# ORNL/DDStore

Hardware: NVIDIA H100
Metric: batch_fetch_GBps (higher is better)
Workload: dtype u8

## Files before the change

ddstore_b200/csrc/kernels.cu:

```cuda
#include <cuda_runtime.h>
#include <stdint.h>
#include <stdio.h>
#include <stdlib.h>
#include <string.h>

#include <algorithm>
#include <atomic>
#include <type_traits>

#include "kernels.h"

namespace {

thread_local char g_cuda_err[512] = "";
std::atomic<unsigned long long> g_launches{0};

#define CUDA_TRY(expr)                                                                                   \
    do {                                                                                                 \
        cudaError_t e__ = (expr);                                                                        \
        if (e__ != cudaSuccess) {                                                                        \
            snprintf(g_cuda_err, sizeof(g_cuda_err), "%s failed: %s (%s:%d)", #expr, cudaGetErrorString(e__), \
                     __FILE__, __LINE__);                                                                \
            return (int)e__ ? (int)e__ : -1;                                                             \
        }                                                                                                \
// ... 537 lines not shown
            continue;
        }
        src[k] = s;
        nbytes[k] = count[k] * vp[k]->row_bytes;
    }
}

__device__ __forceinline__ int64_t warp_incl_scan(int64_t v, int lane) {
#pragma unroll
    for (int d = 1; d < 32; d <<= 1) {
        int64_t o = __shfl_up_sync(0xffffffffu, v, d);
        if (lane >= d) v += o;
    }
    return v;
}
__device__ __forceinline__ int64_t warp_sum(int64_t v) {
#pragma unroll
    for (int d = 16; d > 0; d >>= 1) v += __shfl_xor_sync(0xffffffffu, v, d);
    return v;
}

constexpr int kFopAdd = 0, kFopSwap = 1, kFopCas = 2;

struct GatherArgs {
    ddsk_var_t var;
    const int64_t *starts;
    int64_t count;
    const uint64_t *req_src;
    const int64_t *req_dst;
    const uint32_t *seg_tab;
    PlanSrc plan;
    int64_t *total_out;
    int64_t nreq;
    char *dst;
    int64_t dst_cap;
    int64_t *offsets_out;
    unsigned long long *status;
    unsigned long long status_tag;
    unsigned int *counters;
    union {
        struct {
            char *mdst[DDSK_MAX_MULTI];
            int64_t mcap[DDSK_MAX_MULTI];
            int64_t *moffsets[DDSK_MAX_MULTI];
        };
        struct {
            int64_t pad_slot;
            uint64_t pad_bits;
// ... 32 lines not shown
    uint32_t n;
    uint32_t off;
};

template <int PCAP>
struct PlanView {
    uint32_t src_s, dst_s;
    __device__ __forceinline__ uint64_t s(int64_t i) const { return lds64(src_s + (uint32_t)i * 8u); }
    __device__ __forceinline__ int64_t d(int64_t i) const { return (int64_t)lds32(dst_s + (uint32_t)i * 4u); }
};
template <>
struct PlanView<0> {
    const uint64_t *src;
    const int64_t *dst;
    const uint32_t *seg_tab;
    __device__ __forceinline__ uint64_t s(int64_t i) const { return __ldcg(&src[i]); }
    __device__ __forceinline__ int64_t d(int64_t i) const { return __ldcg(&dst[i]); }
};

__device__ __forceinline__ void pad_lookup(const GatherArgs &a, int64_t idx, uint64_t &src, int64_t &payload) {
    const int64_t ix[1] = {idx};
    uint64_t s[1];
    int64_t nbytes[1];
    plan_many<1>(a.var, a.plan, ix, a.nreq, a.status, a.status_tag, s, nbytes);
    src = s[0];
    payload = min(nbytes[0], a.pad_slot);
}

__device__ __forceinline__ uint4 pad_pattern(uint64_t bits, int el) {
    uint32_t lo, hi;
    if (el == 0) lo = hi = (uint32_t)(bits & 0xFFu) * 0x01010101u;
    else if (el == 1) lo = hi = (uint32_t)(bits & 0xFFFFu) * 0x00010001u;
    else if (el == 2) lo = hi = (uint32_t)bits;
    else {
        lo = (uint32_t)bits;
        hi = (uint32_t)(bits >> 32);
    }
    return make_uint4(lo, hi, lo, hi);
}
__device__ __forceinline__ void pad_store1(char *d, uint64_t bits, int el) {
    if (el == 0) *(uint8_t *)d = (uint8_t)bits;
    else if (el == 1) *(uint16_t *)d = (uint16_t)bits;
    else if (el == 2) *(uint32_t *)d = (uint32_t)bits;
    else *(uint64_t *)d = bits;
}
__device__ __forceinline__ void pad_fill(char *d, int64_t n, uint64_t bits, int el, int lane) {
    int64_t head = (16 - (int64_t)((uint64_t)d & 15u)) & 15;
// ... 29 lines not shown
    int64_t w_dst = 0, w_n = 0;
    uint64_t w_shard;

    __device__ __forceinline__ void load_window(const GatherArgs &a, int lane) {
        win_base = r;
        int64_t idx = r + lane;
        w_src = 0;
        w_dst = 0;
        w_n = 0;
        if (idx < nreq) {
            if constexpr (PAD) {
                int64_t payload;
                pad_lookup(a, idx, w_src, payload);
                w_dst = idx * nb;
                w_n = payload;
            } else if (FIXED && push_n > 0) {
                int p = 0;
                for (int k = 1; k < push_n; k++)
                    if (idx >= push_rbase[k]) p = k;
                const int64_t i = idx - push_rbase[p];
                const int64_t start = ld_relaxed_sys_s64((const int64_t *)(push_win[p] + push_idx_off) + i);
                uint64_t s = 0;
                int owner = 0;
                const int code = dev_locate_owner(a.var, start, a.count, &s, &owner);
                if (code && owner == push_me) {
                    unsigned long long *st = (unsigned long long *)push_win[p] + 3;
                    asm volatile("red.relaxed.sys.global.min.u64 [%0], %1;" ::"l"(st), "l"(((unsigned long long)i << 8) | (unsigned long long)code) : "memory");
                }
                w_src = (code || owner != push_me) ? 0 : s;
                w_dst = idx * nb;
                w_n = nb;
            } else if (FIXED) {
                uint64_t s = 0;
                int code = dev_locate(a.var, a.starts[idx], a.count, &s);
                if (code) report(a.status, a.status_tag, idx, code);
                w_src = code ? 0 : s;
                w_dst = idx * nb;
                w_n = nb;
            } else {
                w_src = pv.s(idx);
                w_dst = pv.d(idx);
                w_n = pv.d(idx + 1) - w_dst;
            }
            if constexpr (PUT) {
                w_shard = w_src;
                w_src = w_src ? (uint64_t)a.dst + (uint64_t)w_dst : 0;
            }
        }
    }

    __device__ __forceinline__ int64_t align_to_var(int64_t pos) const {
        int64_t b = vb[0];
#pragma unroll
        for (int k = 1; k < (VALIGN ? DDSK_MAX_MULTI : 1); k++)
            if (pos >= vb[k]) b = vb[k];
        return b + ((pos - b) & ~(int64_t)7);
    }
// ... 679 lines not shown

struct NoCvt {
    int32_t unused_;
};
template <bool CVT>
using CvtParam = typename std::conditional<CVT, ddsk_cvt_t, NoCvt>::type;

template <int NW, int PCAP, bool CVT = false, bool NORM = false, bool PUT = false>
__device__ __forceinline__ int64_t plan_in_smem(const GatherArgs &a, const PlanView<PCAP> &pv, int64_t *wtot, int warp,
                                                int lane, bool writer, int code = 0) {
    auto out = [&](int64_t x) -> int64_t {
        if constexpr (CVT) return cvt_scale<NORM>(x, code);
        else return x;
    };
    const int64_t nreq = a.nreq;
    const int64_t per_warp = ((nreq + NW * 128 - 1) / (NW * 128)) * 128;
    const int64_t w0 = min(nreq, (int64_t)warp * per_warp), w1 = min(nreq, w0 + per_warp);
    int64_t lane_sum = 0;
    for (int64_t b = w0; b < w1; b += 128) {
        int64_t idx[4], nb[4];
        uint64_t sv[4];
#pragma unroll
        for (int k = 0; k < 4; k++) idx[k] = b + k * 32 + lane;
        plan_many<4, PUT>(a.var, a.plan, idx, w1, a.status, a.status_tag, sv, nb);
#pragma unroll
        for (int k = 0; k < 4; k++) {
            if (idx[k] < w1) {
                sts64(pv.src_s + (uint32_t)idx[k] * 8u, sv[k]);
                sts32(pv.dst_s + (uint32_t)idx[k] * 4u, (uint32_t)min(nb[k], (int64_t)0xFFFFFFFFll));
                lane_sum += nb[k];
            }
        }
    }
    const int64_t wsum = warp_sum(lane_sum);
    if (lane == 0) wtot[warp] = wsum;
    __syncthreads();
    int64_t mine = lane < NW ? wtot[lane] : 0;
    const int64_t T = warp_sum(mine);
    const int64_t base = warp_sum(lane < warp ? mine : 0);
    int64_t run = base;
    for (int64_t b = w0; b < w1; b += 32) {
        const int64_t i = b + lane;
        const int64_t v = i < w1 ? (int64_t)lds32(pv.dst_s + (uint32_t)i * 4u) : 0;
        const int64_t incl = warp_incl_scan(v, lane);
        if (i < w1) {
            sts32(pv.dst_s + (uint32_t)i * 4u, (uint32_t)(run + incl - v));
            if (writer && a.offsets_out) a.offsets_out[i] = out(run + incl - v);
// ... 41 lines not shown
    static_assert(FIXED || !PAD, "a padded batch is a fixed-stride walk");
    static_assert(!PUT || (!CVT && !PAD), "a put writes raw rows");
    static_assert(PUT || !ACC, "an accumulate is a put that adds");
    static_assert((PUT && !ACC) || !FETCH, "a fetch-op is a put that returns the previous rows");
    constexpr int STAGE = CH + 32;
    constexpr bool PUSH = FIXED && !CVT && !PAD && !PUT;
    extern __shared__ __align__(128) unsigned char smem_dyn[];
    __shared__ __align__(8) uint64_t full_bar[NW][S];
    __shared__ __align__(16) PieceDesc desc[NW][S][32];
    __shared__ int64_t wtot[PCAP > 0 ? NW : 1];
    __shared__ int64_t push_rbase[PUSH ? DDSK_MAX_RANKS + 1 : 1];
    __shared__ uint64_t push_win[PUSH ? DDSK_MAX_RANKS : 1];

    const int lane = threadIdx.x & 31;
    const int warp = threadIdx.x >> 5;
    const int64_t gwarp = (int64_t)blockIdx.x * NW + warp;
    const int64_t nwarps = (int64_t)gridDim.x * NW;

    if (lane == 0) {
#pragma unroll
        for (int s = 0; s < S; s++) mbar_init(smem_u32(&full_bar[warp][s]), 1);
        fence_mbar_init();
    }
    uint32_t lut_s = 0;
    if constexpr (CVT) {
        lut_s = smem_u32(smem_dyn) + (uint32_t)(NW * S * STAGE + (PCAP ? PCAP * 12 + 16 : 0));
        for (int i = threadIdx.x; i < c.lut_bytes / 4; i += NW * 32) sts32(lut_s + 4u * (uint32_t)i, c.lut[i]);
        __syncthreads();
    }
    int code0 = 0;
    if constexpr (CVT) code0 = c.code[0];
    if (a.dbg && threadIdx.x == 0) a.dbg[blockIdx.x * 4 + 0] = globaltimer_ns();
    if (a.overlap && !a.wait1_valid) {
        asm volatile("griddepcontrol.wait;" ::: "memory");
        asm volatile("griddepcontrol.launch_dependents;" ::: "memory");
    } else {
        asm volatile("griddepcontrol.launch_dependents;" ::: "memory");
        if (!a.skip_wait) asm volatile("griddepcontrol.wait;" ::: "memory");
    }
    bool gate_open = !(a.overlap && a.wait2_valid);
    auto pass_gate = [&]() {
        if (!gate_open) {
            if (lane == 0) spin_until_done(a.ovl, a.seq - 2u, a.status, a.status_tag, a.nreq);
            __syncwarp();
            gate_open = true;
        }
    };

    ChunkWalker<FIXED, CH, PCAP, CVT, PAD, PUT> w;
    if (!FIXED) {
        if constexpr (PCAP > 0) {
            w.pv.src_s = smem_u32(smem_dyn) + (uint32_t)(NW * S * STAGE);
// ... 64 lines not shown
                    mine_n = ld_relaxed_sys_s64((const int64_t *)ps->win[r] + 1 + par);
                }
                const int64_t incl = warp_incl_scan(mine_n, lane);
                if (r < P) push_rbase[r] = n + incl - mine_n;
                n += __shfl_sync(0xffffffffu, incl, 31);
            }
            if (lane == 0) push_rbase[P] = n;
        }
        __syncthreads();
        w.push_n = P;
        w.push_me = me;
        w.push_par = par;
        w.push_rbase = push_rbase;
        w.push_win = push_win;
        w.push_idx_off = ps->idx_off[par];
    }
    if (a.dbg && threadIdx.x == 0) a.dbg[blockIdx.x * 4 + 1] = globaltimer_ns();
    bool dbg_first = a.dbg != nullptr && warp == 0;
    w.gwarp = gwarp;
    w.nwarps = nwarps;
    w.static_claims = a.tickets == nullptr;
    w.gate_ok = gate_open;
    if constexpr (PAD) w.nb = a.pad_slot;
    else w.nb = (FIXED && a.count <= a.var.lenlist[a.var.nranks - 1]) ? a.count * a.var.row_bytes : 0;
    w.nreq = (FIXED && push) ? push_rbase[w.push_n] : a.nreq;
    if (FIXED) w.T = w.nb * w.nreq;
    bool over = w.T > a.dst_cap;
    const int64_t push_dst_off = (FIXED && push) ? a.push->dst_off[w.push_par] : 0;
    const bool multi = !FIXED && a.plan.nvars > 1;
    int64_t vbase[DDSK_MAX_MULTI + 1];
#pragma unroll
    for (int v = 0; v <= DDSK_MAX_MULTI; v++) vbase[v] = INT64_MAX;
    if (multi) {
        over = false;
#pragma unroll
        for (int v = 0; v < DDSK_MAX_MULTI; v++)
            if (v < a.plan.nvars) vbase[v] = w.pv.d((int64_t)v * a.plan.per_var);
#pragma unroll
        for (int v = 0; v < DDSK_MAX_MULTI; v++)
            if (v < a.plan.nvars) {
                const int64_t endv = v + 1 < a.plan.nvars ? vbase[v + 1] : w.T;
                over |= endv - vbase[v] > a.mcap[v];
            }
        if (PCAP > 0) over |= w.T > 0xFFFFFFFFll;
        if constexpr (CVT) {
            w.valign = true;
#pragma unroll
// ... 46 lines not shown
    {
        if constexpr (PAD) {
            w.seg_bytes = ddsk_fixed_seg_bytes(w.T, w.nb, nwarps, a.min_seg_chunks, CH);
        } else {
        int64_t target = w.T / (nwarps * 8);
        const int64_t unit = (!FIXED && PCAP == 0) ? SEG_GRAIN : (int64_t)CH;
        target = max((int64_t)a.min_seg_chunks * CH, min(target, (int64_t)1 << 20));
        target = max(target, unit);
        if (FIXED && w.nb > 0 && w.nb <= target)
            w.seg_bytes = (target / w.nb) * w.nb;
        else
            w.seg_bytes = (target / unit) * unit;
        }
        w.nseg = w.T > 0 ? (w.T + w.seg_bytes - 1) / w.seg_bytes : 0;
    }
    if (over) {
        if (gwarp == 0 && lane == 0) report(a.status, a.status_tag, a.nreq, DDSK_CODE_CAPACITY);
        w.nseg = 0;
    }

    if (FIXED && !PAD && !push && (w.nb <= 0 || over)) {
        for (int64_t i = gwarp * 32 + lane; i < a.nreq; i += nwarps * 32) {
            uint64_t s;
            int code = dev_locate(a.var, a.starts[i], a.count, &s);
            if (code) report(a.status, a.status_tag, i, code);
        }
    }

    const uint32_t ring = smem_u32(smem_dyn) + (uint32_t)warp * (uint32_t)(S * STAGE);

    uint32_t issued = 0, consumed = 0;
    bool more = w.nseg > 0;
    while (true) {
        while (more && issued - consumed < (uint32_t)(S - 1)) {
            Piece pc;
            const uint32_t total = w.template next_group<STAGE>(a, lane, pc, pass_gate);
            if (total == 0) {
                more = false;
                break;
            }
            const uint32_t st = issued % S;
            const uint32_t bar = smem_u32(&full_bar[warp][st]);
            bulk_wait_read<1>();
            if (lane == 0) mbar_expect_tx(bar, total);
            __syncwarp();
            const uint32_t al = (uint32_t)(pc.src & 15u);
            desc[warp][st][lane].dpos = pc.dpos;
// ... 145 lines not shown
            if (v < a.plan.nvars && a.moffsets[v]) {
                const int64_t basev = w.pv.d((int64_t)v * a.plan.per_var);
                int64_t e = (v * a.plan.per_var + j == a.nreq) ? w.T : w.pv.d((int64_t)v * a.plan.per_var + j);
                if constexpr (CVT) a.moffsets[v][j] = cvt_scale<NORM>(e - basev, c.code[v]);
                else a.moffsets[v][j] = e - basev;
            }
        }
        if constexpr (CVT) {
            if (gwarp == 0 && lane == 0 && a.total_out) {
                int64_t t = 0;
#pragma unroll
                for (int v = 0; v < DDSK_MAX_MULTI; v++)
                    if (v < a.plan.nvars) t += cvt_scale<NORM>((v + 1 < a.plan.nvars ? vbase[v + 1] : w.T) - vbase[v], c.code[v]);
                *a.total_out = t;
            }
        }
    }
    if constexpr (PAD) {
        if (a.pad_lengths || w.nb == 0) {
            for (int64_t i = gwarp * 32 + lane; i < a.nreq; i += nwarps * 32) {
                uint64_t src;
                int64_t payload;
                pad_lookup(a, i, src, payload);
                if (a.pad_lengths) a.pad_lengths[i] = payload / a.var.row_bytes;
            }
        }
    }
    if (FIXED && a.offsets_out && !push) {
        if constexpr (CVT) {
            for (int64_t i = gwarp * 32 + lane; i <= a.nreq; i += nwarps * 32) a.offsets_out[i] = cvt_scale<NORM>(i * w.nb, code0);
        } else {
            for (int64_t i = gwarp * 32 + lane; i <= a.nreq; i += nwarps * 32) a.offsets_out[i] = i * w.nb;
        }
    }

    if (a.dbg && lane == 0) atomicMax(&a.dbg[blockIdx.x * 4 + 3], (unsigned long long)globaltimer_ns());
    if (a.overlap) {
        if (lane == 0) {
            __threadfence();
            const unsigned int slot = a.seq & 3u;
            const unsigned int done = atomicAdd(&a.ovl[slot], 1u);
            if (done == (unsigned int)(nwarps - 1)) {
                a.ovl[slot] = 0;
                a.ovl[8 + slot] = 0;
                if (a.wait_plan) a.plan_word[slot] = 0;
                if (a.wait1_valid) spin_until_done(a.ovl, a.seq - 1u, a.status, a.status_tag, a.nreq);
                __threadfence();
// ... 431 lines not shown
        cfg.numAttrs = 2;
    }
    g_l2_base = nullptr;
    g_l2_bytes = 0;
    CUDA_TRY(cudaLaunchKernelEx(&cfg, kern, args...));
    g_launches++;
    return 0;
}

template <bool FIXED, const Geometry &G, const Geometry &GF>
int launch_kind(const GatherArgs &args, cudaStream_t stream, const ddsk_cvt_t *cvt, bool put, bool acc, bool fop) {
    if (fop) return launch_gather_t<FIXED, GF, false, false, false, true, false, true>(args, stream);
    if (acc) return launch_gather_t<FIXED, G, false, false, false, true, true>(args, stream);
    if (put) return launch_gather_t<FIXED, G, false, false, false, true>(args, stream);
    if (cvt) return cvt_has_norm(cvt) ? launch_gather_t<FIXED, G, true, true>(args, stream, cvt)
                                      : launch_gather_t<FIXED, G, true>(args, stream, cvt);
    return launch_gather_t<FIXED, G>(args, stream);
}

template <bool FIXED>
int launch_gather(const GatherArgs &args, cudaStream_t stream, const ddsk_cvt_t *cvt, bool put = false, bool acc = false,
                  bool fop = false) {
    if constexpr (FIXED) {
        const int64_t request_bytes = args.count < ((int64_t)1 << 20) ? args.count * args.var.row_bytes : INT64_MAX;
        if (!put && !acc && !fop && !cvt && request_bytes < 2048) return launch_gather_t<true, kSmallRows>(args, stream);
    }
    return launch_kind<FIXED, kLargeRows, kFetch>(args, stream, cvt, put, acc, fop);
}

int select_s(int64_t nreq, int64_t cap, const ddsk_cvt_t *cvt) {
    if (!g_smem_plan || cap >= ((int64_t)1 << 32) || nreq > kPlanSmemMax || nreq > g_plan_smem_default) return -1;
    if (nreq <= kPlan4K.pcap) return !cvt || cvt_s_fits_t<kPlan4K>(cvt->lut_bytes) ? 0 : -1;
    return !cvt || cvt_s_fits_t<kPlan8K>(cvt->lut_bytes) ? 1 : -1;
}

int gather_args(GatherArgs &a, const ddsk_var_t *var, const ddsk_scratch_t *scr, int flags) {
    if (int rc = pick_geometry()) return rc;
    memset(&a, 0, sizeof(a));
    a.var = *var;
    a.status = scr->status;
    a.status_tag = scr->status_tag;
    a.counters = scr->counters;
    a.host_mirror = (flags & DDSK_F_MIRROR) ? scr->host_mirror : nullptr;
    a.min_seg_chunks = 1;
    a.overlap = (flags & DDSK_F_OVERLAP) ? 1 : 0;
    a.skip_wait = (flags & DDSK_F_SKIP_WAIT) ? 1 : 0;
    a.wait1_valid = (flags & DDSK_F_PREV1) ? 1 : 0;
    a.wait2_valid = (flags & DDSK_F_PREV2) ? 1 : 0;
    a.seq = scr->ovl_seq;
    a.ovl = scr->ovl;
    a.tickets = a.overlap ? nullptr : scr->counters;
    if (flags & (DDSK_F_ACC | DDSK_F_FOP)) a.acc_type = DDSK_F_ACC_TYPE(flags);
    if (flags & DDSK_F_FOP) {
        a.fop_op = (flags & DDSK_F_FOP_CAS) ? kFopCas : (flags & DDSK_F_FOP_SWAP) ? kFopSwap : kFopAdd;
        a.fop_result = (char *)scr->fop_result;
        a.fop_compare = (const char *)scr->fop_compare;
        a.fop_el = DDSK_F_ACC_TYPE(flags);
    }
    return 0;
}

}
// ... 276 lines not shown
```

ddstore_b200/csrc/kernels.h:

```cpp
#ifndef DDSK_KERNELS_H
#define DDSK_KERNELS_H

#include <stdint.h>

#ifdef __cplusplus
extern "C" {
#endif

#define DDSK_MAX_RANKS 64
#define DDSK_MAX_MULTI 4

typedef struct ddsk_var {
    const void *bases[DDSK_MAX_RANKS];
    int64_t lenlist[DDSK_MAX_RANKS];
    int64_t row_bytes;
    int32_t nranks;
    int32_t pad_;
} ddsk_var_t;

#define DDSK_STATUS_OK 0xFFFFFFFFFFFFFFFFull
#define DDSK_STATUS_ORD_SHIFT 48
#define DDSK_STATUS_REQ_MASK 0xFFFFFFFFFFull
#define DDSK_CODE_START 2
#define DDSK_CODE_COUNT 3
#define DDSK_CODE_CAPACITY 12
#define DDSK_CODE_WATCHDOG 14
#define DDSK_CODE_SAMPLE 15

typedef struct ddsk_scratch {
    unsigned long long *status;
    int64_t *total;
    unsigned int *counters;
    unsigned int *ovl;
    unsigned long long *plan_word;
    unsigned int ovl_seq;
    unsigned long long status_tag;
    uint64_t *req_src;
    int64_t *req_dst;
    int64_t *tile_sums;
    unsigned int plan_tag;
// ... 184 lines not shown
```

ddstore_b200/csrc/store.cpp:

```cpp
#include <cuda_runtime_api.h>
#include <sched.h>
#include <sys/random.h>
#include <unistd.h>

#include <algorithm>
#include <atomic>
#include <condition_variable>
#include <mutex>
#include <thread>
#include <cstdio>
#include <cstdlib>
#include <cstring>
#include <ctime>
#include <map>
#include <set>
#include <string>
#include <vector>

#include "ddstore_b200.h"
#include "internal.h"
#include "kernels.h"
#include "vmm.h"


// ... 137 lines not shown
        src = sp;
        dst = d;
        bytes = n;
        remaining = (int)workers.size();
        gen++;
        cv_go.notify_all();
        cv_done.wait(lk, [&] { return remaining == 0; });
    }
    void stop() {
        {
            std::lock_guard<std::mutex> lk(mu);
            quit = true;
        }
        cv_go.notify_all();
        for (auto &t : workers) t.join();
        workers.clear();
    }
};

struct dds_store {
    dds_comm_t *comm = nullptr;
    int rank = 0, size = 1, device = 0, method = 0;
    cudaStream_t stream = nullptr;
    std::map<std::string, Var> vars;
    std::vector<void *> zombies;
    std::vector<dds_vmm::Block> zombie_blocks;
    unsigned long long token = 0;
    unsigned long long reg_seq = 0;
    ddsk_scratch_t scr;
    int64_t *d_starts = nullptr, *d_counts = nullptr;
    int64_t idx_cap = 0;
    void *d_out = nullptr;
    int64_t out_cap = 0;
    unsigned long long *h_status = nullptr;
    char *h_small = nullptr, *d_small = nullptr;
    struct Queue {
        bool pending = false;
        cudaStream_t pending_stream = nullptr;
        int64_t pending_fixed_total = -1;
        const int64_t *pending_total_ptr = nullptr;
        int pending_cvt = 0;
        bool pending_put = false;
        unsigned int queue_len = 0;
        unsigned int ovl_seq = 1;
        int run_len = 0;
        unsigned long long kept_status = DDSK_STATUS_OK;
        int64_t kept_total = 0;
// ... 205 lines not shown
int entry_var(dds_store *s, const char *name, const int *itemsize, int64_t *total_bytes, int64_t *bad_index, Var **v) {
    clear_error();
    if (bad_index) *bad_index = -1;
    if (total_bytes) *total_bytes = 0;
    if (!s) return fail(DDS_ERR_ARG, "null store");
    *v = find_var(s, name);
    if (!*v) return fail(DDS_ERR_UNKNOWN_VAR, name ? name : "(null)");
    if (itemsize && (*v)->itemsize != *itemsize) return fail(DDS_ERR_DTYPE);
    return DDS_OK;
}

void release_var(Var &v, int rank) {
    for (size_t r = 0; r < v.peer_base.size(); r++) {
        if ((int)r == rank || !v.peer_base[r]) continue;
        if (v.peer_opened[r] == 1) cudaIpcCloseMemHandle(v.peer_base[r]);
        if (v.peer_opened[r] == 2) dds_vmm::release(&v.peer_block[r]);
    }
    v.peer_base.clear();
    v.peer_opened.clear();
    v.peer_block.clear();
}

void free_shard(Var &v) {
    if (v.d_tab) cudaFree(v.d_tab);
    v.d_tab = nullptr;
    if (v.d_norm) cudaFree(v.d_norm);
    v.d_norm = nullptr;
    v.norm_nchan = 0;
    if (v.vmm)
        dds_vmm::release(&v.block);
    else if (v.base)
        cudaFree(v.base);
    v.base = nullptr;
}

int register_var(dds_store *s, const char *name, const void *buffer, int64_t nrows, int disp, int itemsize,
                 int buffer_on_device, bool zero_fill) {
    if (!s || !name) return fail(DDS_ERR_ARG, "null store or name");
    int local_rc = DDS_OK;
    std::string local_err;
    auto note = [&](int rc) {
        if (rc && !local_rc) {
            local_rc = rc;
            local_err = dds_last_error();
        }
    };
// ... 6 lines not shown
    note_cuda(cudaSetDevice(s->device), "cudaSetDevice");
    const bool exists = s->vars.count(name) != 0;
    const unsigned long long seq = s->reg_seq++;

    const size_t payload = local_rc ? 0 : (size_t)nrows * (size_t)disp * (size_t)itemsize;
    size_t alloc = ((payload + 16 + 255) / 256) * 256;
    Var v;
    v.vmm = dds_vmm::available(s->device);
    void *base = nullptr;
    if (!local_rc) {
        if (v.vmm) {
            note(dds_vmm::alloc(s->device, alloc, &v.block));
            if (!local_rc) {
                base = v.block.ptr;
                alloc = v.block.size;
            }
        } else {
            note_cuda(cudaMalloc(&base, alloc), "cudaMalloc (shard)");
            if (local_rc) base = nullptr;
        }
    }
    v.base = base;
    v.bytes = alloc;
    if (base) {
        if (zero_fill || payload == 0) {
            note_cuda(cudaMemsetAsync(base, 0, alloc, s->stream), "cudaMemsetAsync (shard)");
        } else {
            note_cuda(cudaMemsetAsync((char *)base + payload, 0, alloc - payload, s->stream), "cudaMemsetAsync (slack)");
            note_cuda(cudaMemcpyAsync(base, buffer, payload,
                                      buffer_on_device ? cudaMemcpyDeviceToDevice : cudaMemcpyHostToDevice, s->stream),
                      "cudaMemcpyAsync (shard fill)");
        }
        note_cuda(cudaStreamSynchronize(s->stream), "cudaStreamSynchronize (shard fill)");
    }

    PeerRec mine;
    memset(&mine, 0, sizeof(mine));
    mine.nrows = local_rc ? 0 : nrows;
    mine.disp = disp;
    mine.itemsize = itemsize;
    mine.pid = (int32_t)getpid();
    mine.device = s->device;
    mine.raw_ptr = (uint64_t)base;
    mine.host_tag = host_tag();
    mine.alloc_bytes = alloc;
    mine.vmm = v.vmm ? 1 : 0;
    if (s->size > 1 && !v.vmm && base) note_cuda(cudaIpcGetMemHandle(&mine.handle, base), "cudaIpcGetMemHandle");
// ... 97 lines not shown
            if (map_rc) break;
            v.peer_base[(size_t)r] = v.peer_block[(size_t)r].ptr;
            v.peer_opened[(size_t)r] = 2;
        } else {
            v.unprotected_peers = true;
            void *mapped = nullptr;
            cudaError_t e = cudaIpcOpenMemHandle(&mapped, p.handle, cudaIpcMemLazyEnablePeerAccess);
            if (e != cudaSuccess) {
                map_rc = cuda_fail(e, "cudaIpcOpenMemHandle");
                break;
            }
            v.peer_base[(size_t)r] = mapped;
            v.peer_opened[(size_t)r] = 1;
        }
    }
    for (int fd : fds)
        if (fd >= 0) close(fd);
    if (!map_rc && v.vmm) {
        for (int r = 0; r < s->size && !map_rc; r++) {
            const PeerRec &p = all[(size_t)r];
            if (r != s->rank && p.pid == mine.pid && p.device != s->device) map_rc = dds_vmm::grant(&v.block, p.device);
        }
    }
    const std::string keep_err = dds_last_error();
    int brc = dds_comm_barrier(s->comm);

    if (map_rc || bad_disp || bad_item || exists) {
        release_var(v, s->rank);
        if (base) {
            if (v.vmm)
                s->zombie_blocks.push_back(v.block);
            else
                s->zombies.push_back(base);
        }
        if (local_rc) {
            g_err = local_err;
            return local_rc;
        }
        if (map_rc) {
            g_err = keep_err;
            return map_rc;
        }
        if (bad_disp) return fail(DDS_ERR_DISP);
        if (bad_item) return fail(DDS_ERR_DTYPE);
        return fail(DDS_ERR_EXISTS, name);
    }
    memset(&v.kv, 0, sizeof(v.kv));
    for (int r = 0; r < s->size; r++) {
        v.kv.bases[r] = v.peer_base[(size_t)r];
        v.kv.lenlist[r] = v.lenlist[(size_t)r];
    }
    v.kv.row_bytes = (int64_t)disp * (int64_t)itemsize;
    v.kv.nranks = s->size;
    if (s->db_enabled && s->d_vars && s->next_var_id < dds_store::kMaxDbVars) {
        if (cudaMemcpy(&s->d_vars[s->next_var_id], &v.kv, sizeof(ddsk_var_t), cudaMemcpyHostToDevice) == cudaSuccess)
            v.id = s->next_var_id++;
        (void)cudaGetLastError();
    }
    s->vars.emplace(v.name, std::move(v));
    return brc;
}

int64_t sat_mul(int64_t a, int64_t b) {
    int64_t r;
    return __builtin_mul_overflow(a, b, &r) ? INT64_MAX : r;
}
int64_t sat_add(int64_t a, int64_t b) {
    int64_t r;
    return __builtin_add_overflow(a, b, &r) ? INT64_MAX : r;
}

int cvt_in_log2(int code) { return DDSK_CVT_IN_LOG2(code); }
int cvt_out_log2(int code) { return DDSK_CVT_OUT_LOG2(code); }
int64_t cvt_to_out(int64_t p, int code) {
    if (p == INT64_MAX) return p;
    return sat_mul(p >> cvt_in_log2(code), (int64_t)1 << cvt_out_log2(code));
// ... 37 lines not shown
    q.pending = false;
    q.pending_put = false;
    break_run(s);
    cudaStream_t st = q.pending_stream;
    CU(cudaMemcpyAsync(&s->h_status[0], s->scr.status, 8, cudaMemcpyDeviceToHost, st));
    if (q.pending_fixed_total < 0 && q.pending_total_ptr)
        CU(cudaMemcpyAsync(&s->h_status[1], q.pending_total_ptr, 8, cudaMemcpyDeviceToHost, st));
    CU(cudaStreamSynchronize(st));
    q.kept_total = q.pending_fixed_total >= 0 ? q.pending_fixed_total : cvt_to_out((int64_t)s->h_status[1], q.pending_cvt);
    const unsigned long long stw = s->h_status[0];
    if (stw != DDSK_STATUS_OK) {
        if (q.kept_status == DDSK_STATUS_OK) q.kept_status = stw;
        rearm_status(s, st);
    }
    return DDS_OK;
}

struct Call {
    cudaStream_t st;
    bool no_sync, chain;
};

int begin_call(dds_store *s, void *cuda_stream, bool no_sync, Call *c) {
    CU(cudaSetDevice(s->device));
    c->st = cuda_stream ? (cudaStream_t)cuda_stream : s->stream;
    c->no_sync = no_sync;
    c->chain = s->q.pending && no_sync && c->st == s->q.pending_stream;
    if (s->q.pending && !c->chain) return drain_pending(s);
    return DDS_OK;
}

void note_empty_async(dds_store *s, const Call &c) {
    if (!c.no_sync) return;
    if (s->q.pending) {
        s->q.pending_fixed_total = 0;
        s->q.pending_cvt = DDSK_CVT_NONE;
    } else {
        s->q.kept_total = 0;
    }
}

constexpr unsigned int kQueueMax = 0xFFFF;
int launch_flags(dds_store *s, const Call &c, bool ovl, bool plan_slot, int *kflags, ddsk_scratch_t *scr) {
    dds_store::Queue &q = s->q;
    bool chain = c.chain;
    if (chain && q.queue_len >= kQueueMax) {
        if (int rc = drain_pending(s)) return rc;
// ... 1326 lines not shown
```

ddstore_b200/store.py:

```python
import ctypes as C

import numpy as np

from . import _capi
from .comm import as_dds_comm

_NP_OK = {np.dtype(np.int32), np.dtype(np.int64), np.dtype(np.uint8), np.dtype(np.float32),
          np.dtype(np.float64), np.dtype(np.bool_)}
_TORCH_OK = {"torch.int32", "torch.int64", "torch.uint8", "torch.float32", "torch.float64", "torch.bool"}
_TORCH_HALF = {"torch.bfloat16", "torch.float16"}

_CVT_CODES = {("float32", "bfloat16"): _capi.CVT_F32_BF16, ("float32", "float16"): _capi.CVT_F32_F16,
              ("float64", "float32"): _capi.CVT_F64_F32, ("uint8", "bfloat16"): _capi.CVT_U8_LUT16,
              ("uint8", "float16"): _capi.CVT_U8_LUT16, ("uint8", "float32"): _capi.CVT_U8_LUT32}
_NORM_CODES = {("float32", "float32"): _capi.CVT_NORM_F32_F32, ("float32", "bfloat16"): _capi.CVT_NORM_F32_BF16,
               ("float32", "float16"): _capi.CVT_NORM_F32_F16, ("float64", "float32"): _capi.CVT_NORM_F64_F32,
               ("uint8", "float32"): _capi.CVT_NORM_U8_F32, ("uint8", "bfloat16"): _capi.CVT_NORM_U8_BF16,
               ("uint8", "float16"): _capi.CVT_NORM_U8_F16}
_U8_NORM = (_capi.CVT_NORM_U8_F32, _capi.CVT_NORM_U8_BF16, _capi.CVT_NORM_U8_F16)
_default_luts = {}


def _dtype_name(dt):
    s = str(dt)
    if s.startswith("torch."):
        return s[len("torch."):]
    if s in ("bfloat16", "float16"):
        return s
    return str(np.dtype(dt))


def _conversion(src_dtype, out_dtype, lut, normalize=False):
    import torch
# ... 72 lines not shown
        t = torch.tensor([iv], dtype=dtype)
    n = t.element_size()
    return int(t.view(getattr(torch, _INT_VIEW[n])).item()) & ((1 << (8 * n)) - 1)


def _lut_bits(t):
    import torch
    t = t.detach().reshape(-1).cpu().contiguous()
    return t.view(torch.int16 if t.element_size() == 2 else torch.int32).numpy().copy()


class _Buf:

    def __init__(self, arr, writable=False, half_ok=False):
        self.keep = arr
        if isinstance(arr, np.ndarray):
            assert arr.flags.c_contiguous
            if arr.dtype not in _NP_OK:
                raise NotImplementedError
            self.ptr, self.on_device = arr.ctypes.data, 0
            self.shape, self.itemsize, self.size = arr.shape, arr.dtype.itemsize, arr.size
        elif hasattr(arr, "data_ptr") and hasattr(arr, "element_size"):
            assert arr.is_contiguous()
            if str(arr.dtype) not in _TORCH_OK and not (half_ok and str(arr.dtype) in _TORCH_HALF):
                raise NotImplementedError
            self.ptr, self.on_device = arr.data_ptr(), 1 if arr.is_cuda else 0
            self.shape, self.itemsize, self.size = tuple(arr.shape), arr.element_size(), arr.numel()
        elif hasattr(arr, "__cuda_array_interface__"):
            cai = arr.__cuda_array_interface__
            if cai.get("strides") is not None:
                raise ValueError("device array must be C-contiguous")
            dt = np.dtype(cai["typestr"])
            if dt not in _NP_OK:
                raise NotImplementedError
            self.ptr, self.on_device = cai["data"][0], 1
            self.shape, self.itemsize = tuple(cai["shape"]), dt.itemsize
            self.size = int(np.prod(self.shape, dtype=np.int64))
        else:
            raise TypeError(f"unsupported array type {type(arr).__name__}")
        self.nbytes = self.size * self.itemsize


class _DevMem:

    def __init__(self, ptr, nbytes):
        self.__cuda_array_interface__ = {"shape": (int(nbytes),), "typestr": "|u1", "data": (int(ptr), False), "version": 2}


def _i64(x):
    return np.ascontiguousarray(x, dtype=np.int64)


class PyDDStore:
    def __init__(self, comm=None, method=0, device=None):
        self._L = _capi.lib()
        self._comm = as_dds_comm(comm)
        self._h = self._L.dds_create(self._comm.handle, -1 if device is None else int(device), int(method))
        if not self._h:
            raise RuntimeError(_capi.last_error())
        self.rank, self.size = self._L.dds_rank(self._h), self._L.dds_size(self._h)
        self._itemsize = {}
        self._cname = {}
        self._rowbytes = {}
        self.last_bad_index = -1

    def add(self, name, arr):
        b = _Buf(arr)
        nrows = b.shape[0]
        disp = b.size // b.shape[0] if b.shape[0] else int(np.prod(b.shape[1:], dtype=np.int64))
        _capi.raise_for(self._L.dds_add(self._h, name.encode(), b.ptr, nrows, disp, b.itemsize, b.on_device))

    def get(self, name, arr, start=0):
        cn = self._cname.get(name)
        if cn is None:
            cn = self._cname[name] = name.encode()
        if type(arr) is np.ndarray:
            assert arr.flags.c_contiguous
            if arr.dtype not in _NP_OK:
                raise NotImplementedError
            rc = self._L.dds_get(self._h, cn, int(start), arr.shape[0], arr.dtype.itemsize, arr.ctypes.data, 0)
        else:
            b = _Buf(arr, writable=True)
            rc = self._L.dds_get(self._h, cn, int(start), b.shape[0], b.itemsize, b.ptr, b.on_device)
        if rc:
            _capi.raise_for(rc)

    def epoch_begin(self):
# ... 52 lines not shown
            nreq = starts.numel()
            sp = starts.data_ptr()
            cp = counts.data_ptr() if counts is not None else None
            keep = (starts, counts)
        else:
            sa = _i64(starts)
            nreq = sa.size
            sp = sa.ctypes.data
            ca = _i64(counts) if counts is not None else None
            cp = ca.ctypes.data if ca is not None else None
            keep = (sa, ca)
        flags = (_capi.IDX_ON_DEVICE if s_dev else 0) | (_capi.DST_ON_DEVICE if ob.on_device else 0)
        if not wait:
            flags |= _capi.NO_SYNC | (_capi.OVERLAP if overlap else 0)
        if pad_rows is not None:
            return self._padded(name, False, sp, cp, nreq, out, ob, cv, pad_rows, pad_value, lengths, flags, stream,
                                (keep, lut_keep))
        op = None
        if offsets is not None:
            fb = _Buf(offsets, writable=True)
            if fb.on_device != ob.on_device or fb.itemsize != 8 or fb.size < nreq + 1:
                raise ValueError("offsets must be int64[len(starts)+1] with the same residency as out")
            op = fb.ptr
        total, bad = C.c_int64(0), C.c_int64(-1)
        if cv is None:
            rc = self._L.dds_get_batch(self._h, name.encode(), sp, cp, 1 if count is None else int(count), nreq,
                                       itemsize, ob.ptr, ob.nbytes, op, flags,
                                       self._stream_arg(stream), C.byref(total), C.byref(bad))
        else:
            rc = self._L.dds_get_batch_convert(self._h, name.encode(), sp, cp, 1 if count is None else int(count), nreq,
                                               ob.ptr, ob.nbytes, op, flags, self._stream_arg(stream), C.byref(cv),
                                               C.byref(total), C.byref(bad))
        del keep, lut_keep
        self.last_bad_index = bad.value
        _capi.raise_for(rc)
        return total.value

    def put_batch(self, name, starts, counts=None, src=None, count=None, stream=None, wait=True):
        sb, keep_src = self._put_src(name, src)
        s_dev = hasattr(starts, "data_ptr") and getattr(starts, "is_cuda", False)
        if s_dev:
            nreq, sp = starts.numel(), starts.data_ptr()
            cp = counts.data_ptr() if counts is not None else None
            keep = (starts, counts)
        else:
            sa = _i64(starts)
            ca = _i64(counts) if counts is not None else None
            nreq, sp, cp = sa.size, sa.ctypes.data, ca.ctypes.data if ca is not None else None
            keep = (sa, ca)
        flags = _capi.SRC_ON_DEVICE | (_capi.IDX_ON_DEVICE if s_dev else 0) | (0 if wait else _capi.NO_SYNC)
        total, bad = C.c_int64(0), C.c_int64(-1)
        rc = self._L.dds_put_batch(self._h, name.encode(), sp, cp, 1 if count is None else int(count), nreq, sb.itemsize,
                                   sb.ptr, sb.nbytes, flags, self._stream_arg(stream), C.byref(total), C.byref(bad))
        del keep, keep_src
        self.last_bad_index = bad.value
# ... 346 lines not shown
        c_offs = None
        if offsets is not None:
            fbs = [_Buf(f, writable=True) for f in offsets]
            c_offs = (C.c_void_p * nv)(*[f.ptr for f in fbs])
        totals = (C.c_int64 * nv)()
        bad = C.c_int64(-1)
        if cvs is None:
            rc = self._L.dds_get_samples_multi(self._h, nv, c_names, sp, nreq, c_dsts, c_caps, c_offs, flags,
                                               self._stream_arg(stream), totals, C.byref(bad))
        else:
            rc = self._L.dds_get_samples_multi_convert(self._h, nv, c_names, sp, nreq, c_dsts, c_caps, c_offs, flags,
                                                       self._stream_arg(stream), cvs, totals, C.byref(bad))
            del lut_keep
        del keep
        self.last_bad_index = bad.value
        _capi.raise_for(rc)
        return [totals[v] for v in range(nv)] if wait else None

    @staticmethod
    def _stream_arg(stream):
        if stream is None:
            return None
        h = int(stream)
        return C.c_void_p(h if h != 0 else 1)

    def wait(self):
        total, bad = C.c_int64(0), C.c_int64(-1)
        rc = self._L.dds_batch_wait(self._h, C.byref(total), C.byref(bad))
        self.last_bad_index = bad.value
        _capi.raise_for(rc)
        return total.value

    def query(self, name):
        vi = _capi.VarInfo()
        _capi.raise_for(self._L.dds_query(self._h, name.encode(), C.byref(vi)))
        return {"itemsize": vi.itemsize, "disp": vi.disp, "nranks": vi.nranks, "fence_active": bool(vi.fence_active),
                "local_nrows": vi.local_nrows, "total_nrows": vi.total_nrows,
                "lenlist": [vi.lenlist[i] for i in range(vi.nranks)], "local_base": vi.local_base}

    def synth_fill(self, name, seed):
        _capi.raise_for(self._L.dds_synth_fill(self._h, name.encode(), int(seed)))

    def synth_verify(self, name, packed, starts, counts=None, count=1, offsets=None, seed=0, stream=None):
        res = (C.c_uint64 * 66)()
        _capi.raise_for(self._L.dds_synth_verify(
            self._h, name.encode(), packed.data_ptr(), starts.data_ptr(), counts.data_ptr() if counts is not None else None,
            int(count), offsets.data_ptr() if offsets is not None else None, starts.numel(), int(seed),
# ... 14 lines not shown
```

Baseline: 1455.

## Pass var descriptor by device pointer and trim per-call host overhead

Replaces the large by-value ddsk_var_t kernel argument with a device-resident copy that is loaded into a shared-memory struct at block start, which shrinks the kernel parameter block. It also avoids a redundant cudaSetDevice per call, caches encoded names and ctypes out-params, and speeds up the torch dtype check in Python. In exchange each block does a small global load and an extra __syncthreads at startup, and a device allocation is added per variable.

```diff
diff --git a/ddstore_b200/csrc/kernels.cu b/ddstore_b200/csrc/kernels.cu
--- a/ddstore_b200/csrc/kernels.cu
+++ b/ddstore_b200/csrc/kernels.cu
@@ -583,8 +583,12 @@
 
 constexpr int kFopAdd = 0, kFopSwap = 1, kFopCas = 2;
 
+__shared__ ddsk_var_t s_var;
+
 struct GatherArgs {
-    ddsk_var_t var;
+    const ddsk_var_t *var;
+    int64_t row_bytes;
+    int32_t nranks;
     const int64_t *starts;
     int64_t count;
     const uint64_t *req_src;
@@ -663,7 +667,7 @@
     const int64_t ix[1] = {idx};
     uint64_t s[1];
     int64_t nbytes[1];
-    plan_many<1>(a.var, a.plan, ix, a.nreq, a.status, a.status_tag, s, nbytes);
+    plan_many<1>(s_var, a.plan, ix, a.nreq, a.status, a.status_tag, s, nbytes);
     src = s[0];
     payload = min(nbytes[0], a.pad_slot);
 }
@@ -739,7 +743,7 @@
                 const int64_t start = ld_relaxed_sys_s64((const int64_t *)(push_win[p] + push_idx_off) + i);
                 uint64_t s = 0;
                 int owner = 0;
-                const int code = dev_locate_owner(a.var, start, a.count, &s, &owner);
+                const int code = dev_locate_owner(s_var, start, a.count, &s, &owner);
                 if (code && owner == push_me) {
                     unsigned long long *st = (unsigned long long *)push_win[p] + 3;
                     asm volatile("red.relaxed.sys.global.min.u64 [%0], %1;" ::"l"(st), "l"(((unsigned long long)i << 8) | (unsigned long long)code) : "memory");
@@ -749,7 +753,7 @@
                 w_n = nb;
             } else if (FIXED) {
                 uint64_t s = 0;
-                int code = dev_locate(a.var, a.starts[idx], a.count, &s);
+                int code = dev_locate(s_var, a.starts[idx], a.count, &s);
                 if (code) report(a.status, a.status_tag, idx, code);
                 w_src = code ? 0 : s;
                 w_dst = idx * nb;
@@ -1475,7 +1479,7 @@
         uint64_t sv[4];
 #pragma unroll
         for (int k = 0; k < 4; k++) idx[k] = b + k * 32 + lane;
-        plan_many<4, PUT>(a.var, a.plan, idx, w1, a.status, a.status_tag, sv, nb);
+        plan_many<4, PUT>(s_var, a.plan, idx, w1, a.status, a.status_tag, sv, nb);
 #pragma unroll
         for (int k = 0; k < 4; k++) {
             if (idx[k] < w1) {
@@ -1563,12 +1567,22 @@
         for (int s = 0; s < S; s++) mbar_init(smem_u32(&full_bar[warp][s]), 1);
         fence_mbar_init();
     }
+    if (a.var) {
+        for (int r = threadIdx.x; r < a.nranks; r += NW * 32) {
+            s_var.bases[r] = a.var->bases[r];
+            s_var.lenlist[r] = a.var->lenlist[r];
+        }
+        if (threadIdx.x == 0) {
+            s_var.row_bytes = a.row_bytes;
+            s_var.nranks = a.nranks;
+        }
+    }
     uint32_t lut_s = 0;
     if constexpr (CVT) {
         lut_s = smem_u32(smem_dyn) + (uint32_t)(NW * S * STAGE + (PCAP ? PCAP * 12 + 16 : 0));
         for (int i = threadIdx.x; i < c.lut_bytes / 4; i += NW * 32) sts32(lut_s + 4u * (uint32_t)i, c.lut[i]);
-        __syncthreads();
-    }
+    }
+    __syncthreads();
     int code0 = 0;
     if constexpr (CVT) code0 = c.code[0];
     if (a.dbg && threadIdx.x == 0) a.dbg[blockIdx.x * 4 + 0] = globaltimer_ns();
@@ -1679,7 +1693,7 @@
     w.static_claims = a.tickets == nullptr;
     w.gate_ok = gate_open;
     if constexpr (PAD) w.nb = a.pad_slot;
-    else w.nb = (FIXED && a.count <= a.var.lenlist[a.var.nranks - 1]) ? a.count * a.var.row_bytes : 0;
+    else w.nb = (FIXED && a.count <= s_var.lenlist[a.nranks - 1]) ? a.count * a.row_bytes : 0;
     w.nreq = (FIXED && push) ? push_rbase[w.push_n] : a.nreq;
     if (FIXED) w.T = w.nb * w.nreq;
     bool over = w.T > a.dst_cap;
@@ -1772,7 +1786,7 @@
     if (FIXED && !PAD && !push && (w.nb <= 0 || over)) {
         for (int64_t i = gwarp * 32 + lane; i < a.nreq; i += nwarps * 32) {
             uint64_t s;
-            int code = dev_locate(a.var, a.starts[i], a.count, &s);
+            int code = dev_locate(s_var, a.starts[i], a.count, &s);
             if (code) report(a.status, a.status_tag, i, code);
         }
     }
@@ -1964,7 +1978,7 @@
                 uint64_t src;
                 int64_t payload;
                 pad_lookup(a, i, src, payload);
-                if (a.pad_lengths) a.pad_lengths[i] = payload / a.var.row_bytes;
+                if (a.pad_lengths) a.pad_lengths[i] = payload / a.row_bytes;
             }
         }
     }
@@ -2442,7 +2456,7 @@
 int launch_gather(const GatherArgs &args, cudaStream_t stream, const ddsk_cvt_t *cvt, bool put = false, bool acc = false,
                   bool fop = false) {
     if constexpr (FIXED) {
-        const int64_t request_bytes = args.count < ((int64_t)1 << 20) ? args.count * args.var.row_bytes : INT64_MAX;
+        const int64_t request_bytes = args.count < ((int64_t)1 << 20) ? args.count * args.row_bytes : INT64_MAX;
         if (!put && !acc && !fop && !cvt && request_bytes < 2048) return launch_gather_t<true, kSmallRows>(args, stream);
     }
     return launch_kind<FIXED, kLargeRows, kFetch>(args, stream, cvt, put, acc, fop);
@@ -2457,7 +2471,9 @@
 int gather_args(GatherArgs &a, const ddsk_var_t *var, const ddsk_scratch_t *scr, int flags) {
     if (int rc = pick_geometry()) return rc;
     memset(&a, 0, sizeof(a));
-    a.var = *var;
+    a.var = var->dev;
+    a.row_bytes = var->row_bytes;
+    a.nranks = var->nranks;
     a.status = scr->status;
     a.status_tag = scr->status_tag;
     a.counters = scr->counters;
diff --git a/ddstore_b200/csrc/kernels.h b/ddstore_b200/csrc/kernels.h
--- a/ddstore_b200/csrc/kernels.h
+++ b/ddstore_b200/csrc/kernels.h
@@ -16,6 +16,7 @@
     int64_t row_bytes;
     int32_t nranks;
     int32_t pad_;
+    const struct ddsk_var *dev;
 } ddsk_var_t;
 
 #define DDSK_STATUS_OK 0xFFFFFFFFFFFFFFFFull
diff --git a/ddstore_b200/csrc/store.cpp b/ddstore_b200/csrc/store.cpp
--- a/ddstore_b200/csrc/store.cpp
+++ b/ddstore_b200/csrc/store.cpp
@@ -183,7 +183,7 @@
     dds_comm_t *comm = nullptr;
     int rank = 0, size = 1, device = 0, method = 0;
     cudaStream_t stream = nullptr;
-    std::map<std::string, Var> vars;
+    std::map<std::string, Var, std::less<>> vars;
     std::vector<void *> zombies;
     std::vector<dds_vmm::Block> zombie_blocks;
     unsigned long long token = 0;
@@ -435,6 +435,8 @@
 }
 
 void free_shard(Var &v) {
+    if (v.kv.dev) cudaFree((void *)v.kv.dev);
+    v.kv.dev = nullptr;
     if (v.d_tab) cudaFree(v.d_tab);
     v.d_tab = nullptr;
     if (v.d_norm) cudaFree(v.d_norm);
@@ -487,7 +489,11 @@
     }
     v.base = base;
     v.bytes = alloc;
+    memset(&v.kv, 0, sizeof(v.kv));
     if (base) {
+        ddsk_var_t *d_kv = nullptr;
+        note_cuda(cudaMalloc((void **)&d_kv, sizeof(ddsk_var_t)), "cudaMalloc (window)");
+        v.kv.dev = d_kv;
         if (zero_fill || payload == 0) {
             note_cuda(cudaMemsetAsync(base, 0, alloc, s->stream), "cudaMemsetAsync (shard)");
         } else {
@@ -631,11 +637,22 @@
             if (r != s->rank && p.pid == mine.pid && p.device != s->device) map_rc = dds_vmm::grant(&v.block, p.device);
         }
     }
+    if (!map_rc && base) {
+        for (int r = 0; r < s->size; r++) {
+            v.kv.bases[r] = v.peer_base[(size_t)r];
+            v.kv.lenlist[r] = v.lenlist[(size_t)r];
+        }
+        v.kv.row_bytes = (int64_t)disp * (int64_t)itemsize;
+        v.kv.nranks = s->size;
+        const cudaError_t e = cudaMemcpy((void *)v.kv.dev, &v.kv, sizeof(ddsk_var_t), cudaMemcpyHostToDevice);
+        if (e != cudaSuccess) map_rc = cuda_fail(e, "cudaMemcpy (window)");
+    }
     const std::string keep_err = dds_last_error();
     int brc = dds_comm_barrier(s->comm);
 
     if (map_rc || bad_disp || bad_item || exists) {
         release_var(v, s->rank);
+        if (v.kv.dev) cudaFree((void *)v.kv.dev);
         if (base) {
             if (v.vmm)
                 s->zombie_blocks.push_back(v.block);
@@ -654,13 +671,6 @@
         if (bad_item) return fail(DDS_ERR_DTYPE);
         return fail(DDS_ERR_EXISTS, name);
     }
-    memset(&v.kv, 0, sizeof(v.kv));
-    for (int r = 0; r < s->size; r++) {
-        v.kv.bases[r] = v.peer_base[(size_t)r];
-        v.kv.lenlist[r] = v.lenlist[(size_t)r];
-    }
-    v.kv.row_bytes = (int64_t)disp * (int64_t)itemsize;
-    v.kv.nranks = s->size;
     if (s->db_enabled && s->d_vars && s->next_var_id < dds_store::kMaxDbVars) {
         if (cudaMemcpy(&s->d_vars[s->next_var_id], &v.kv, sizeof(ddsk_var_t), cudaMemcpyHostToDevice) == cudaSuccess)
             v.id = s->next_var_id++;
@@ -744,7 +754,8 @@
 };
 
 int begin_call(dds_store *s, void *cuda_stream, bool no_sync, Call *c) {
-    CU(cudaSetDevice(s->device));
+    int cur = -1;
+    if (cudaGetDevice(&cur) != cudaSuccess || cur != s->device) CU(cudaSetDevice(s->device));
     c->st = cuda_stream ? (cudaStream_t)cuda_stream : s->stream;
     c->no_sync = no_sync;
     c->chain = s->q.pending && no_sync && c->st == s->q.pending_stream;
diff --git a/ddstore_b200/store.py b/ddstore_b200/store.py
--- a/ddstore_b200/store.py
+++ b/ddstore_b200/store.py
@@ -9,6 +9,15 @@
           np.dtype(np.float64), np.dtype(np.bool_)}
 _TORCH_OK = {"torch.int32", "torch.int64", "torch.uint8", "torch.float32", "torch.float64", "torch.bool"}
 _TORCH_HALF = {"torch.bfloat16", "torch.float16"}
+_torch_sets = []
+
+
+def _torch_dtypes():
+    if not _torch_sets:
+        import torch
+        ok = {getattr(torch, n[len("torch."):]) for n in _TORCH_OK}
+        _torch_sets.extend([ok, ok | {getattr(torch, n[len("torch."):]) for n in _TORCH_HALF}])
+    return _torch_sets
 
 _CVT_CODES = {("float32", "bfloat16"): _capi.CVT_F32_BF16, ("float32", "float16"): _capi.CVT_F32_F16,
               ("float64", "float32"): _capi.CVT_F64_F32, ("uint8", "bfloat16"): _capi.CVT_U8_LUT16,
@@ -127,10 +136,10 @@
             self.shape, self.itemsize, self.size = arr.shape, arr.dtype.itemsize, arr.size
         elif hasattr(arr, "data_ptr") and hasattr(arr, "element_size"):
             assert arr.is_contiguous()
-            if str(arr.dtype) not in _TORCH_OK and not (half_ok and str(arr.dtype) in _TORCH_HALF):
+            if arr.dtype not in (_torch_sets or _torch_dtypes())[1 if half_ok else 0]:
                 raise NotImplementedError
             self.ptr, self.on_device = arr.data_ptr(), 1 if arr.is_cuda else 0
-            self.shape, self.itemsize, self.size = tuple(arr.shape), arr.element_size(), arr.numel()
+            self.shape, self.itemsize, self.size = arr.shape, arr.element_size(), arr.numel()
         elif hasattr(arr, "__cuda_array_interface__"):
             cai = arr.__cuda_array_interface__
             if cai.get("strides") is not None:
@@ -168,6 +177,8 @@
         self._cname = {}
         self._rowbytes = {}
         self.last_bad_index = -1
+        self._total, self._bad = C.c_int64(0), C.c_int64(-1)
+        self._total_p, self._bad_p = C.byref(self._total), C.byref(self._bad)
 
     def add(self, name, arr):
         b = _Buf(arr)
@@ -266,15 +277,18 @@
             if fb.on_device != ob.on_device or fb.itemsize != 8 or fb.size < nreq + 1:
                 raise ValueError("offsets must be int64[len(starts)+1] with the same residency as out")
             op = fb.ptr
-        total, bad = C.c_int64(0), C.c_int64(-1)
+        total, bad = self._total, self._bad
+        cn = self._cname.get(name)
+        if cn is None:
+            cn = self._cname[name] = name.encode()
         if cv is None:
-            rc = self._L.dds_get_batch(self._h, name.encode(), sp, cp, 1 if count is None else int(count), nreq,
+            rc = self._L.dds_get_batch(self._h, cn, sp, cp, 1 if count is None else int(count), nreq,
                                        itemsize, ob.ptr, ob.nbytes, op, flags,
-                                       self._stream_arg(stream), C.byref(total), C.byref(bad))
-        else:
-            rc = self._L.dds_get_batch_convert(self._h, name.encode(), sp, cp, 1 if count is None else int(count), nreq,
+                                       self._stream_arg(stream), self._total_p, self._bad_p)
+        else:
+            rc = self._L.dds_get_batch_convert(self._h, cn, sp, cp, 1 if count is None else int(count), nreq,
                                                ob.ptr, ob.nbytes, op, flags, self._stream_arg(stream), C.byref(cv),
-                                               C.byref(total), C.byref(bad))
+                                               self._total_p, self._bad_p)
         del keep, lut_keep
         self.last_bad_index = bad.value
         _capi.raise_for(rc)
@@ -667,7 +681,7 @@
         if stream is None:
             return None
         h = int(stream)
-        return C.c_void_p(h if h != 0 else 1)
+        return h if h != 0 else 1
 
     def wait(self):
         total, bad = C.c_int64(0), C.c_int64(-1)
```

After: 1457, median of 6. Within noise of the previous version (+0.2%).
